# rsinghlab/GNN-Tumor-Seg

Hardware: AMD Instinct MI355X
Metric: supervoxel-graphs/sec training, 7xSAGE-pool-256, 15k-node graphs (higher is better)
Workload: dtype f32; 1 GPU; C2: 7xGraphSAGE-pool-256 (8 SAGEConv), fwd+weighted-CE+bwd+AdamW, 4 x 15000-node/86350-edge lattice graphs per GPU, 4-chan feat, fp32; global_batch=4, nodes_per_batch=60000, edges_per_batch=345400, parallelism=dp1

## Files before the change

gnn-tumor-seg_amd/csrc/gts_options.hip:

```cpp
#include "gts_gemm_args.h"
#include "gts_rows.h"

namespace gts {
namespace {

struct Option { int32_t id; int* knob; bool (*legal)(int32_t); };

const Option kOptions[] = {
    {GTS_OPT_GEMM_TILE, &g_fwd_variant, [](int32_t v) { return v == -1 || v == -2 || v == 1 || v == 3 || v == 5 || v == 8 || v == 10; }},
    {GTS_OPT_IGRAD_TILE, &g_igrad_variant, [](int32_t v) { return v == -1 || v == 1 || v == 3 || v == 5 || v == 8 || v == 10; }},
    {GTS_OPT_WGRAD_TILE, &g_wgrad_variant, [](int32_t v) { return v == -1 || v == 1 || v == 2 || v == 4 || v == 6; }},
    {GTS_OPT_GEMM_SCHED, &g_gemm_sched, nullptr},
    {GTS_OPT_PANEL_ROWS, &g_panel_rows, nullptr},
    {GTS_OPT_SPMM_ROWS_PER_WAVE, &g_spmm_seq, nullptr},
    {GTS_OPT_SPMM_STREAMING, &g_spmm_nt, nullptr},
    {GTS_OPT_PROJECT_STREAMING, &g_project_nt, nullptr},
    {GTS_OPT_CLUSTER_STREAMING, &g_cluster_nt, nullptr},
    {GTS_OPT_CLUSTER_DEALING, &g_cluster_dealing, [](int32_t v) { return v >= 0 && v <= 2; }},
    {GTS_OPT_CLUSTER_RING, &g_cluster_ring, nullptr},
    {GTS_OPT_CLUSTER_PER_CU, &g_cluster_per_cu, nullptr},
    {GTS_OPT_CLUSTER_CONSUMERS, &g_cluster_consumers, nullptr},
    {GTS_OPT_GAT_WALK, &g_gat_walk, nullptr},
    {GTS_OPT_GAT_CLUSTER_WAVES, &g_gat_cluster_waves, nullptr},
    {GTS_OPT_GAT_CLUSTER_GROUP, &g_gat_cluster_group, nullptr},
    {GTS_OPT_GAT_CLUSTER_DEALING, &g_gat_cluster_dealing, [](int32_t v) { return v == 0 || v == 1; }},
};

const Option* find_option(int32_t id) {
  for (const Option& o : kOptions)
    if (o.id == id) return &o;
  return nullptr;
}

}
}

extern "C" int32_t gts_set_option(int32_t option, int32_t value) {
  const gts::Option* o = gts::find_option(option);
  if (o == nullptr || (o->legal != nullptr && !o->legal(value))) return GTS_ERR_ARGKIND;
  *o->knob = value;
  return GTS_OK;
}

extern "C" int32_t gts_get_option(int32_t option) {
  const gts::Option* o = gts::find_option(option);
  return o != nullptr ? *o->knob : INT32_MIN;
}
```

gnn-tumor-seg_amd/csrc/gts_rows.h:

```cpp
#pragma once
#include <type_traits>

#include "gts_common.h"

namespace gts {

constexpr int kUnroll = 8;

__device__ __forceinline__ float mad(float w, float v, float acc) { return __builtin_fmaf(w, v, acc); }

typedef float v2f __attribute__((ext_vector_type(2)));
constexpr float kEluSplit = -0.35f, kLog2e = 1.44269504088896340736f;
constexpr float kEluC2 = 0.5f, kEluC3 = 1.0f / 6.0f, kEluC4 = 1.0f / 24.0f, kEluC5 = 1.0f / 120.0f, kEluC6 = 1.0f / 720.0f,
                kEluC7 = 1.0f / 5040.0f;
__device__ __forceinline__ float elu_expm1(float x) {
  float q = __builtin_fmaf(kEluC7, x, kEluC6);
  q = __builtin_fmaf(q, x, kEluC5);
  q = __builtin_fmaf(q, x, kEluC4);
  q = __builtin_fmaf(q, x, kEluC3);
  q = __builtin_fmaf(q, x, kEluC2);
  const float small = __builtin_fmaf(x * x, q, x);
  const float large = __builtin_amdgcn_exp2f(x * kLog2e) - 1.0f;
  return x < kEluSplit ? large : small;
}
// ... 29 lines not shown
    body(active ? c : 0, active);
  }
}

template <int N>
using IC = std::integral_constant<int, N>;

template <int LPR, typename Body>
__device__ __forceinline__ void for_chunks(int beg, int end, Body&& body) {
  if constexpr (LPR == kWave) {
    int k = beg;
    for (; k + kUnroll <= end; k += kUnroll) body(IC<kUnroll>{}, k);
    switch (end - k) {
      case 1: body(IC<1>{}, k); break;
      case 2: body(IC<2>{}, k); break;
      case 3: body(IC<3>{}, k); break;
      case 4: body(IC<4>{}, k); break;
      case 5: body(IC<5>{}, k); break;
      case 6: body(IC<6>{}, k); break;
      case 7: body(IC<7>{}, k); break;
      default: break;
    }
  } else {
    for (int k = beg; k < end; k += kUnroll) body(IC<kUnroll>{}, k);
  }
}

template <int LPR, int CNT>
struct Chunk {
  int reg;
  const int32_t* __restrict__ p;
  int k, last;
  __device__ __forceinline__ Chunk(const int32_t* __restrict__ arr, int k_, int end) : p(arr), k(k_), last(end - 1) {
    if constexpr (LPR == kWave) {
      const int lane = threadIdx.x & (kWave - 1);
      reg = lane < CNT ? arr[k_ + lane] : 0;
    } else {
      reg = 0;
    }
  }
  __device__ __forceinline__ int operator[](int j) const {
    if constexpr (LPR == kWave) {
      return __builtin_amdgcn_readlane(reg, j);
    } else {
      return p[min(k + j, last)];
    }
  }
  __device__ __forceinline__ bool valid(int j) const {
    if constexpr (LPR == kWave) return true;
    return k + j <= last;
  }
};

inline int g_spmm_seq = 0;
inline int g_project_nt = 1;
inline int g_spmm_nt = -1;
inline int g_cluster_nt = -1;
inline int g_gat_walk = 1;
inline int g_cluster_ring = 0;
inline int g_cluster_per_cu = 0;
inline int g_gat_cluster_waves = 0;
inline int g_cluster_dealing = 0;
inline int g_gat_cluster_dealing = 0;
inline int g_gat_cluster_group = 0;
inline int g_cluster_consumers = 0;

inline int pick_seq(int64_t n_rows, int rows_per_wave_step, int preferred) {
  if (g_spmm_seq > 0) return g_spmm_seq;
  if (preferred > 0) return preferred;
  const int64_t steps = (n_rows + rows_per_wave_step - 1) / rows_per_wave_step;
  int seq = 1;
  while (seq < 4 && steps / (seq * 2) >= 8192) seq *= 2;
  return seq;
}

struct Geometry {
  int vec, lpr, seq;
  dim3 grid;
};

inline Geometry make_geometry(int64_t n_rows, int64_t n_feat, int preferred_seq = 0) {
  Geometry g;
  g.vec = (n_feat % 4 == 0) ? 4 : 1;
  g.lpr = lanes_per_row(n_feat / g.vec);
  const int rows_per_step = kWave / g.lpr;
  g.seq = pick_seq(n_rows, rows_per_step, preferred_seq);
  const int64_t rows_per_block = static_cast<int64_t>(rows_per_step) * g.seq * kWavesPerBlock;
  g.grid = dim3(static_cast<unsigned>((n_rows + rows_per_block - 1) / rows_per_block));
  return g;
}

inline bool bad_shape(int64_t n_rows, int64_t n_feat) {
  return n_rows < 0 || n_feat <= 0 || n_rows >= (1LL << 31) || n_feat >= (1LL << 24);
}

}

#define GTS_DISPATCH_LPR(VEC_, LPR_VAL, ...)                \
  switch (LPR_VAL) {                                        \
    case 1: { constexpr int LPR = 1; __VA_ARGS__; } break;  \
    case 2: { constexpr int LPR = 2; __VA_ARGS__; } break;  \
    case 4: { constexpr int LPR = 4; __VA_ARGS__; } break;  \
    case 8: { constexpr int LPR = 8; __VA_ARGS__; } break;  \
    case 16: { constexpr int LPR = 16; __VA_ARGS__; } break; \
    case 32: { constexpr int LPR = 32; __VA_ARGS__; } break; \
    default: { constexpr int LPR = 64; __VA_ARGS__; } break; \
  }

#define GTS_DISPATCH_GEOM(G, ...)                                   \
  if ((G).vec == 4) {                                               \
    constexpr int VEC = 4;                                          \
    GTS_DISPATCH_LPR(4, (G).lpr, __VA_ARGS__)                       \
  } else {                                                          \
    constexpr int VEC = 1;                                          \
    GTS_DISPATCH_LPR(1, (G).lpr, __VA_ARGS__)                       \
  }
```

gnn-tumor-seg_amd/csrc/gts_spmm.hip:

```cpp
#include "gts_rows.h"

namespace gts {
namespace {

template <int ARGB>
struct ArgTraits;
template <>
struct ArgTraits<1> {
  using T = uint8_t;
  static constexpr int kNone = 0xFF;
};
template <>
struct ArgTraits<4> {
  using T = int32_t;
  static constexpr int kNone = -1;
};

template <int VEC, int ARGB>
__device__ __forceinline__ void store_slots(void* arg, size_t off, const int (&slot)[VEC]) {
  if constexpr (ARGB == 1) {
    uint8_t* p = static_cast<uint8_t*>(arg) + off;
    if constexpr (VEC == 4) {
      const uint32_t w = (slot[0] & 0xFF) | ((slot[1] & 0xFF) << 8) | ((slot[2] & 0xFF) << 16) |
                         (static_cast<uint32_t>(slot[3] & 0xFF) << 24);
      *reinterpret_cast<uint32_t*>(p) = w;
    } else {
      p[0] = static_cast<uint8_t>(slot[0]);
    }
  } else if constexpr (ARGB == 4) {
    int32_t* p = static_cast<int32_t*>(arg) + off;
    if constexpr (VEC == 4) {
      *reinterpret_cast<int4*>(p) = make_int4(slot[0], slot[1], slot[2], slot[3]);
    } else {
      p[0] = slot[0];
    }
  }
}

template <int VEC, int ARGB>
__device__ __forceinline__ void load_slots(const void* arg, size_t off, int (&slot)[VEC]) {
  if constexpr (ARGB == 1) {
    const uint8_t* p = static_cast<const uint8_t*>(arg) + off;
    if constexpr (VEC == 4) {
      const uint32_t w = *reinterpret_cast<const uint32_t*>(p);
      slot[0] = w & 0xFF;
      slot[1] = (w >> 8) & 0xFF;
      slot[2] = (w >> 16) & 0xFF;
      slot[3] = w >> 24;
    } else {
      slot[0] = p[0];
    }
  } else {
    const int32_t* p = static_cast<const int32_t*>(arg) + off;
    if constexpr (VEC == 4) {
      const int4 w = *reinterpret_cast<const int4*>(p);
      slot[0] = w.x, slot[1] = w.y, slot[2] = w.z, slot[3] = w.w;
    } else {
      slot[0] = p[0];
    }
  }
}

template <int VEC, int LPR, int ARGB>
__global__ __launch_bounds__(kBlock) void spmm_max_fwd_kernel(
    const int32_t* __restrict__ indptr, const int32_t* __restrict__ indices,
    const float* __restrict__ x, float* __restrict__ out, void* __restrict__ arg, int n_dst,
    int n_feat, int seq, int nt, int relu_input) {
  for (int s = 0; s < seq; ++s) {
    const int v = owned_row<LPR>(s, seq, n_dst);
    if (v < 0) continue;
    const int beg = indptr[v], end = indptr[v + 1];
    for_columns<VEC, LPR>(n_feat, [&](int c, bool active) {
      float best[VEC];
      int slot[VEC];
#pragma unroll
      for (int t = 0; t < VEC; ++t) best[t] = -INFINITY, slot[t] = -1;
      for_chunks<LPR>(beg, end, [&](auto cnt_c, int k) {
        constexpr int CNT = decltype(cnt_c)::value;
        const Chunk<LPR, CNT> src(indices, k, end);
        Vec<VEC> val[CNT];
#pragma unroll
        for (int j = 0; j < CNT; ++j)
          val[j] = Vec<VEC>::load(x + static_cast<size_t>(src[j]) * n_feat + c);
#pragma unroll
        for (int j = 0; j < CNT; ++j) {
          if (src.valid(j)) {
#pragma unroll
            for (int t = 0; t < VEC; ++t) {
              if (best[t] < val[j].v[t]) best[t] = val[j].v[t], slot[t] = k + j - beg;
            }
          }
        }
      });
      Vec<VEC> o;
#pragma unroll
      for (int t = 0; t < VEC; ++t) {
        const bool dead = isinf(best[t]);
        o.v[t] = dead ? 0.0f : best[t];
        slot[t] = (dead || (relu_input && !(best[t] > 0.0f))) ? -1 : slot[t];
      }
      const size_t off = static_cast<size_t>(v) * n_feat + c;
      if (active) {
        if (nt & 1) o.store_nt(out + off); else o.store(out + off);
        if constexpr (ARGB != 0) store_slots<VEC, ARGB>(arg, off, slot);
      }
    });
  }
}

template <int VEC, int LPR, int ARGB>
__global__ __launch_bounds__(kBlock) void spmm_max_bwd_kernel(
    const int32_t* __restrict__ t_indptr, const int32_t* __restrict__ t_indices,
    const int32_t* __restrict__ t_slot, const float* __restrict__ gout,
    const void* __restrict__ arg, const float* __restrict__ relu_src, float* __restrict__ gx,
    int n_src, int n_feat, int seq, int nt) {
  for (int s = 0; s < seq; ++s) {
    const int u = owned_row<LPR>(s, seq, n_src);
    if (u < 0) continue;
    const int beg = t_indptr[u], end = t_indptr[u + 1];
    for_columns<VEC, LPR>(n_feat, [&](int c, bool active) {
      float acc[VEC];
#pragma unroll
      for (int t = 0; t < VEC; ++t) acc[t] = 0.0f;
      for_chunks<LPR>(beg, end, [&](auto cnt_c, int k) {
        constexpr int CNT = decltype(cnt_c)::value;
        const Chunk<LPR, CNT> dst(t_indices, k, end);
        const Chunk<LPR, CNT> slt(t_slot, k, end);
        Vec<VEC> g[CNT];
        int win[CNT][VEC];
        int want[CNT];
#pragma unroll
        for (int j = 0; j < CNT; ++j) {
          const size_t off = static_cast<size_t>(dst[j]) * n_feat + c;
          want[j] = slt[j];
          g[j] = Vec<VEC>::load(gout + off);
          load_slots<VEC, ARGB>(arg, off, win[j]);
        }
#pragma unroll
        for (int j = 0; j < CNT; ++j) {
          if (dst.valid(j)) {
#pragma unroll
            for (int t = 0; t < VEC; ++t) acc[t] += (win[j][t] == want[j]) ? g[j].v[t] : 0.0f;
          }
        }
      });
      const size_t off = static_cast<size_t>(u) * n_feat + c;
      Vec<VEC> o;
      if (relu_src != nullptr) {
        const Vec<VEC> p = (nt & 2) ? Vec<VEC>::load_nt(relu_src + off) : Vec<VEC>::load(relu_src + off);
#pragma unroll
        for (int t = 0; t < VEC; ++t) o.v[t] = p.v[t] > 0.0f ? acc[t] : 0.0f;
      } else {
#pragma unroll
        for (int t = 0; t < VEC; ++t) o.v[t] = acc[t];
      }
      if (active) { if (nt & 1) o.store_nt(gx + off); else o.store(gx + off); }
    });
  }
}

constexpr int kLowRank = 4, kLowRankFeat = 256;

template <int ARGB>
__global__ __launch_bounds__(kBlock) void spmm_max_bwd_lowrank_kernel(
    const int32_t* __restrict__ t_indptr, const int32_t* __restrict__ t_indices,
    const int32_t* __restrict__ t_slot, const float* __restrict__ g, const float* __restrict__ w,
    const void* __restrict__ arg, float* __restrict__ gx, int n_src, int nt) {
  constexpr int VEC = 4, LPR = kWave, R = kLowRank, F = kLowRankFeat;
  const int u = owned_row<LPR>(0, 1, n_src);
  if (u < 0) return;
  const int c = VEC * (threadIdx.x & (kWave - 1));
  Vec<VEC> wk[R];
#pragma unroll
  for (int k = 0; k < R; ++k) wk[k] = Vec<VEC>::load(w + k * F + c);
  const int beg = t_indptr[u], end = t_indptr[u + 1];
  float acc[VEC];
#pragma unroll
  for (int t = 0; t < VEC; ++t) acc[t] = 0.0f;
  for_chunks<LPR>(beg, end, [&](auto cnt_c, int k) {
    constexpr int CNT = decltype(cnt_c)::value;
    const Chunk<LPR, CNT> dst(t_indices, k, end);
    const Chunk<LPR, CNT> slt(t_slot, k, end);
    Vec<R> gr[CNT];
    int win[CNT][VEC];
    int want[CNT];
#pragma unroll
    for (int j = 0; j < CNT; ++j) {
      const size_t d = static_cast<size_t>(dst[j]);
      want[j] = slt[j];
      gr[j] = Vec<R>::load(g + d * R);
      load_slots<VEC, ARGB>(arg, d * F + c, win[j]);
    }
#pragma unroll
    for (int j = 0; j < CNT; ++j) {
#pragma unroll
      for (int t = 0; t < VEC; ++t) {
        float v = 0.0f;
#pragma unroll
        for (int q = 0; q < R; ++q) v = __builtin_fmaf(gr[j].v[q], wk[q].v[t], v);
        acc[t] += (win[j][t] == want[j]) ? v : 0.0f;
      }
    }
  });
  Vec<VEC> o;
#pragma unroll
  for (int t = 0; t < VEC; ++t) o.v[t] = acc[t];
  const size_t off = static_cast<size_t>(u) * F + c;
  if (nt & 1) o.store_nt(gx + off); else o.store(gx + off);
}

template <int VEC, int LPR, bool DIV_IN>
__global__ __launch_bounds__(kBlock) void spmm_sum_kernel(
    const int32_t* __restrict__ indptr, const int32_t* __restrict__ indices,
    const float* __restrict__ x, float* __restrict__ out, const float* __restrict__ div_in,
    const float* __restrict__ div_out, const float* __restrict__ accum, int add_self, int n_out, int n_feat,
    int seq) {
  for (int s = 0; s < seq; ++s) {
    const int v = owned_row<LPR>(s, seq, n_out);
    if (v < 0) continue;
    const int beg = indptr[v], end = indptr[v + 1];
    for_columns<VEC, LPR>(n_feat, [&](int c, bool active) {
      float acc[VEC];
#pragma unroll
      for (int t = 0; t < VEC; ++t) acc[t] = 0.0f;
      for_chunks<LPR>(beg, end, [&](auto cnt_c, int k) {
        constexpr int CNT = decltype(cnt_c)::value;
        const Chunk<LPR, CNT> src(indices, k, end);
        Vec<VEC> val[CNT];
        float d[CNT];
#pragma unroll
        for (int j = 0; j < CNT; ++j) {
          const int u = src[j];
          d[j] = DIV_IN ? div_in[u] : 1.0f;
          val[j] = Vec<VEC>::load(x + static_cast<size_t>(u) * n_feat + c);
        }
#pragma unroll
        for (int j = 0; j < CNT; ++j) {
          if (src.valid(j)) {
#pragma unroll
            for (int t = 0; t < VEC; ++t) acc[t] += DIV_IN ? val[j].v[t] / d[j] : val[j].v[t];
          }
        }
      });
      const size_t off = static_cast<size_t>(v) * n_feat + c;
      if (add_self) {
        const Vec<VEC> self = Vec<VEC>::load(x + off);
        const float d = DIV_IN ? div_in[v] : 1.0f;
#pragma unroll
        for (int t = 0; t < VEC; ++t) acc[t] += DIV_IN ? self.v[t] / d : self.v[t];
      }
      Vec<VEC> o;
      const float dv = div_out != nullptr ? div_out[v] : 1.0f;
#pragma unroll
      for (int t = 0; t < VEC; ++t) o.v[t] = div_out != nullptr ? acc[t] / dv : acc[t];
      if (accum != nullptr) {
        const Vec<VEC> other = Vec<VEC>::load(accum + off);
#pragma unroll
        for (int t = 0; t < VEC; ++t) o.v[t] = other.v[t] + o.v[t];
      }
      if (active) o.store(out + off);
    });
  }
}

}
}

extern "C" int32_t gts_spmm_max_fwd_f32(const int32_t* indptr, const int32_t* indices,
                                        const float* x, float* out, void* arg,
                                        int32_t arg_bytes, int32_t relu_input, int64_t n_dst,
                                        int64_t n_feat, void* stream) {
  using namespace gts;
  if (!indptr || !x || !out || (arg_bytes != 0 && !arg)) return GTS_ERR_NULL;
  if (bad_shape(n_dst, n_feat)) return GTS_ERR_SHAPE;
  if (arg_bytes != 0 && arg_bytes != 1 && arg_bytes != 4) return GTS_ERR_ARGKIND;
  if (n_dst == 0) return GTS_OK;
  const Geometry g = make_geometry(n_dst, n_feat, 2);
  const int nt = g_spmm_nt < 0 ? 1 : g_spmm_nt;
  hipStream_t st = static_cast<hipStream_t>(stream);
  const int nd = static_cast<int>(n_dst), nf = static_cast<int>(n_feat);
  GTS_DISPATCH_GEOM(g, {
    if (arg_bytes == 0)
      spmm_max_fwd_kernel<VEC, LPR, 0><<<g.grid, kBlock, 0, st>>>(indptr, indices, x, out, arg, nd, nf, g.seq, nt, relu_input);
    else if (arg_bytes == 1)
      spmm_max_fwd_kernel<VEC, LPR, 1><<<g.grid, kBlock, 0, st>>>(indptr, indices, x, out, arg, nd, nf, g.seq, nt, relu_input);
    else
      spmm_max_fwd_kernel<VEC, LPR, 4><<<g.grid, kBlock, 0, st>>>(indptr, indices, x, out, arg, nd, nf, g.seq, nt, relu_input);
  })
  return launch_status();
}

extern "C" int32_t gts_spmm_max_bwd_f32(const int32_t* t_indptr, const int32_t* t_indices,
                                        const int32_t* t_slot, const float* gout,
                                        const void* arg, int32_t arg_bytes,
                                        const float* relu_src, float* gx, int64_t n_src,
                                        int64_t n_feat, void* stream) {
  using namespace gts;
  if (!t_indptr || !gout || !arg || !gx) return GTS_ERR_NULL;
  if (bad_shape(n_src, n_feat)) return GTS_ERR_SHAPE;
  if (arg_bytes != 1 && arg_bytes != 4) return GTS_ERR_ARGKIND;
  if (n_src == 0) return GTS_OK;
  const Geometry g = make_geometry(n_src, n_feat, 1);
  const int nt = g_spmm_nt < 0 ? 0 : g_spmm_nt;
  hipStream_t st = static_cast<hipStream_t>(stream);
  const int ns = static_cast<int>(n_src), nf = static_cast<int>(n_feat);
  GTS_DISPATCH_GEOM(g, {
    if (arg_bytes == 1)
      spmm_max_bwd_kernel<VEC, LPR, 1><<<g.grid, kBlock, 0, st>>>(t_indptr, t_indices, t_slot, gout, arg, relu_src, gx, ns, nf, g.seq, nt);
    else
      spmm_max_bwd_kernel<VEC, LPR, 4><<<g.grid, kBlock, 0, st>>>(t_indptr, t_indices, t_slot, gout, arg, relu_src, gx, ns, nf, g.seq, nt);
  })
  return launch_status();
}

extern "C" int32_t gts_spmm_max_bwd_lowrank_f32(const int32_t* t_indptr, const int32_t* t_indices,
                                                const int32_t* t_slot, const float* g, const float* w,
                                                const void* arg, int32_t arg_bytes, float* gx, int64_t n_src,
                                                int64_t n_feat, int64_t rank, void* stream) {
  using namespace gts;
  if (!t_indptr || !g || !w || !arg || !gx) return GTS_ERR_NULL;
  if (bad_shape(n_src, n_feat) || n_feat != kLowRankFeat || rank != kLowRank) return GTS_ERR_SHAPE;
  if (arg_bytes != 1 && arg_bytes != 4) return GTS_ERR_ARGKIND;
  if (n_src == 0) return GTS_OK;
  const int nt = g_spmm_nt < 0 ? 0 : g_spmm_nt;
  hipStream_t st = static_cast<hipStream_t>(stream);
  const unsigned grid = static_cast<unsigned>((n_src + kWavesPerBlock - 1) / kWavesPerBlock);
  const int ns = static_cast<int>(n_src);
  if (arg_bytes == 1)
    spmm_max_bwd_lowrank_kernel<1><<<grid, kBlock, 0, st>>>(t_indptr, t_indices, t_slot, g, w, arg, gx, ns, nt);
  else
    spmm_max_bwd_lowrank_kernel<4><<<grid, kBlock, 0, st>>>(t_indptr, t_indices, t_slot, g, w, arg, gx, ns, nt);
  return launch_status();
}

extern "C" int32_t gts_spmm_sum_f32(const int32_t* indptr, const int32_t* indices,
                                    const float* x, float* out, const float* div_in,
                                    const float* div_out, const float* accum, int32_t add_self,
                                    int64_t n_out, int64_t n_feat, void* stream) {
  using namespace gts;
  if (!indptr || !x || !out) return GTS_ERR_NULL;
  if (bad_shape(n_out, n_feat)) return GTS_ERR_SHAPE;
  if (n_out == 0) return GTS_OK;
  const Geometry g = make_geometry(n_out, n_feat);
  hipStream_t st = static_cast<hipStream_t>(stream);
  const int no = static_cast<int>(n_out), nf = static_cast<int>(n_feat);
  GTS_DISPATCH_GEOM(g, {
    if (div_in != nullptr)
      spmm_sum_kernel<VEC, LPR, true><<<g.grid, kBlock, 0, st>>>(indptr, indices, x, out, div_in, div_out, accum, add_self, no, nf, g.seq);
    else
      spmm_sum_kernel<VEC, LPR, false><<<g.grid, kBlock, 0, st>>>(indptr, indices, x, out, div_in, div_out, accum, add_self, no, nf, g.seq);
  })
  return launch_status();
}
```

gnn-tumor-seg_amd/gts/ops.py:

```python
import ctypes

import torch

from . import _lib
from ._lib import check, current_stream, ptr, require_device
from ._operands import StreamBuffers, expect, f32, scratch
from .graph import _DeviceSchedule

_ARG_DTYPE = {0: torch.uint8, 1: torch.uint8, 4: torch.int32}

KERNEL_TIMERS = {}
INSTRUMENTED = False


def _timed(name, launch):
    timer = KERNEL_TIMERS.get(name)
    return timer(launch) if timer is not None else launch()


_counters = StreamBuffers(torch.int32, zeroed=True)
_COUNTER_BYTES = 4 * _lib.const("GTS_CLUSTER_COUNTER_WORDS")


def cluster_counters(device):
# ... 38 lines not shown
    return g.dev_schedule(which)


def spmm_max_bwd(g, gout, arg, relu_src=None):
    gout = gout.contiguous()
    f32(gout, relu_src)
    require_device(gout, arg, relu_src)
    d = g.dev()
    if gout.dim() != 2 or gout.shape[0] != g.n:
        raise _lib.GtsError(f"gradient must be [graph nodes = {g.n}, F], got {tuple(gout.shape)}")
    n, f = g.n, gout.shape[1]
    expect(arg, (n, f), "arg")
    expect(relu_src, (n, f), "relu_src")
    if arg.dtype != _ARG_DTYPE[g.arg_bytes]:
        raise _lib.GtsError(f"arg dtype {arg.dtype} does not belong to this graph ({_ARG_DTYPE[g.arg_bytes]})")
    gx = torch.empty((n, f), dtype=torch.float32, device=gout.device)
    lib = _lib.load()
    ds = _cluster_schedule(g, "out", n, f, arg.element_size()) if relu_src is None else None
    if ds is not None:
        def launch():
            return lib.gts_spmm_max_bwd_cluster_f32(*_DeviceSchedule.launch_args(ds), ptr(gout), ptr(arg), 1, ptr(gx), n, f,
                                                    ptr(cluster_counters(gout.device)), current_stream())
    else:
        def launch():
            return lib.gts_spmm_max_bwd_f32(ptr(d.t_indptr), ptr(d.t_indices), ptr(d.t_slot), ptr(gout),
                                            ptr(arg), arg.element_size(), ptr(relu_src), ptr(gx), n, f,
                                            current_stream())

    check(_timed("spmm_max_bwd_f256", launch) if f == 256 else launch(), "gts_spmm_max_bwd_f32")
    return gx


def lowrank_bwd_applies(grad, w, arg):
    return grad.shape[1] == 4 and tuple(w.shape) == (4, 256) and arg.element_size() == 1


def spmm_max_bwd_lowrank(g, grad, w, arg):
    grad, w = grad.contiguous(), w.contiguous()
    f32(grad, w)
    require_device(grad, w, arg)
    d = g.dev()
    n = g.n
    if grad.dim() != 2 or grad.shape != (n, 4) or tuple(w.shape) != (4, 256):
        raise _lib.GtsError(f"spmm_max_bwd_lowrank takes a gradient [graph nodes = {n}, 4] and weights [4, 256], "
                            f"got {tuple(grad.shape)} and {tuple(w.shape)}")
    expect(arg, (n, 256), "arg")
    if arg.dtype != _ARG_DTYPE[g.arg_bytes]:
        raise _lib.GtsError(f"arg dtype {arg.dtype} does not belong to this graph ({_ARG_DTYPE[g.arg_bytes]})")
    gx = torch.empty((n, 256), dtype=torch.float32, device=grad.device)
    check(_lib.load().gts_spmm_max_bwd_lowrank_f32(ptr(d.t_indptr), ptr(d.t_indices), ptr(d.t_slot), ptr(grad), ptr(w),
                                                   ptr(arg), arg.element_size(), ptr(gx), n, 256, 4, current_stream()),
          "gts_spmm_max_bwd_lowrank_f32")
    return gx


def spmm_sum_raw(g, x, transposed=False, div_in=None, div_out=None, add_self=False, accum=None):
    x = x.contiguous()
    f32(x, div_in, div_out, accum)
    require_device(x, div_in, div_out, accum)
    d = g.dev()
    indptr, indices = (d.t_indptr, d.t_indices) if transposed else (d.indptr, d.indices)
    n = g.n
    if x.dim() != 2 or x.shape[0] != n:
        raise _lib.GtsError(f"features must be [graph nodes = {n}, F], got {tuple(x.shape)}")
    f = x.shape[1]
    expect(div_in, (n,), "div_in")
    expect(div_out, (n,), "div_out")
    expect(accum, (n, f), "accum")
    out = torch.empty_like(x)
    check(_lib.load().gts_spmm_sum_f32(ptr(indptr), ptr(indices), ptr(x), ptr(out), ptr(div_in), ptr(div_out),
                                       ptr(accum), 1 if add_self else 0, n, f, current_stream()), "gts_spmm_sum_f32")
    return out


class _SpMMMax(torch.autograd.Function):
    @staticmethod
    def forward(ctx, g, x):
        out, arg = spmm_max_fwd(g, x, want_arg=True)
        ctx.g = g
        ctx.save_for_backward(arg)
        return out

    @staticmethod
    def backward(ctx, gout):
        (arg,) = ctx.saved_tensors
        return None, spmm_max_bwd(ctx.g, gout, arg)


class _SpMMReduce(torch.autograd.Function):

    @staticmethod
    def forward(ctx, g, x, mode):
        ctx.g, ctx.mode = g, mode
        d = g.dev()
        if mode == "sum":
            return spmm_sum_raw(g, x)
        if mode == "mean":
            return spmm_sum_raw(g, x, div_out=d.deg_clamped)
        if mode == "gcn":
            return spmm_sum_raw(g, x, div_out=d.deg_plus1, add_self=True)
        raise ValueError(mode)

    @staticmethod
    def backward(ctx, gout):
        g, mode = ctx.g, ctx.mode
        d = g.dev()
# ... 1012 lines not shown
```

include/gts_hip.h:

```cpp
#ifndef GTS_HIP_H
#define GTS_HIP_H

#include <stdint.h>

#ifdef __cplusplus
extern "C" {
#endif

#define GTS_OK 0
#define GTS_ERR_NULL (-1)
#define GTS_ERR_SHAPE (-2)
#define GTS_ERR_ARGKIND (-3)

int32_t gts_abi_version(void);
const char* gts_error_string(int32_t code);

int32_t gts_spmm_max_fwd_f32(const int32_t* indptr, const int32_t* indices, const float* x,
                             float* out, void* arg, int32_t arg_bytes, int32_t relu_input,
                             int64_t n_dst, int64_t n_feat, void* stream);

int32_t gts_spmm_max_bwd_f32(const int32_t* t_indptr, const int32_t* t_indices,
                             const int32_t* t_slot, const float* gout, const void* arg,
                             int32_t arg_bytes, const float* relu_src, float* gx,
                             int64_t n_src, int64_t n_feat, void* stream);
int32_t gts_spmm_max_bwd_lowrank_f32(const int32_t* t_indptr, const int32_t* t_indices,
                                     const int32_t* t_slot, const float* g, const float* w, const void* arg,
                                     int32_t arg_bytes, float* gx, int64_t n_src, int64_t n_feat,
                                     int64_t rank, void* stream);

int64_t gts_cluster_record_words(int32_t max_rows, int32_t max_srcs, int32_t loc_words, int32_t with_tag);
int32_t gts_cluster_schedule(const int32_t* indptr, const int32_t* indices, const int32_t* t_indptr,
                             const int32_t* t_indices, const int32_t* edge_tag, int64_t n_rows,
                             int32_t max_rows, int32_t max_srcs, int32_t max_edges, int32_t* rec,
                             int64_t rec_capacity, int64_t* n_clusters, int64_t* n_staged,
                             int32_t* max_cluster_edges);
int64_t gts_cluster_lds_bytes(int32_t max_rows, int32_t max_srcs, int32_t loc_words, int32_t kind);
int32_t gts_spmm_max_fwd_cluster_f32(const int32_t* rec, int64_t n_clusters, int32_t max_rows, int32_t max_srcs,
                                     int32_t loc_words, const float* x, float* out, void* arg,
                                     int32_t arg_bytes, int32_t relu_input, int64_t n_rows, int64_t n_feat,
                                     uint32_t* counters, void* stream);
int32_t gts_spmm_max_bwd_cluster_f32(const int32_t* rec, int64_t n_clusters, int32_t max_rows, int32_t max_srcs,
                                     int32_t loc_words, const float* gout, const void* arg, int32_t arg_bytes,
                                     float* gx, int64_t n_rows, int64_t n_feat, uint32_t* counters, void* stream);
#define GTS_CLUSTER_COUNTER_WORDS 256
int32_t gts_cluster_uses_counters(int64_t n_clusters, int32_t max_rows, int32_t max_srcs, int32_t loc_words, int32_t backward);

int32_t gts_spmm_sum_f32(const int32_t* indptr, const int32_t* indices, const float* x,
                         float* out, const float* div_in, const float* div_out, const float* accum,
                         int32_t add_self, int64_t n_out, int64_t n_feat, void* stream);

int32_t gts_gat_fwd_f32(const int32_t* indptr, const int32_t* indices, const float* ft,
                        const float* el, const float* er, float negative_slope, const float* bias,
                        const float* residual, int32_t activation, float* out, float* attn,
                        int64_t n, int64_t heads, int64_t dim, void* stream);
int32_t gts_gat_scores_f32(const float* ft, const float* attn_l, const float* attn_r, float* el,
                           float* er, int64_t n, int64_t heads, int64_t dim, void* stream);

int32_t gts_gat_bwd_edge_f32(const int32_t* indptr, const int32_t* indices, const float* ft,
                             const float* el, const float* er, const float* attn,
                             const float* gout, float negative_slope, float* ge, float* ger,
                             int64_t n, int64_t heads, int64_t dim, void* stream);
int32_t gts_gat_bwd_src_f32(const int32_t* t_indptr, const int32_t* t_indices,
                            const int32_t* t_pos, const float* attn, const float* ge,
                            const float* gout, const float* attn_l, const float* attn_r,
                            const float* ger, float* gft, float* gel, int64_t n, int64_t heads,
                            int64_t dim, void* stream);
int64_t gts_gat_reduce_workspace(int64_t n, int64_t cols);
int32_t gts_gat_act_bwd_f32(const float* gout, const float* out, int32_t activation, float* g_pre,
                            float* g_bias, float* workspace, int64_t workspace_bytes, int64_t n,
                            int64_t cols, void* stream);
int32_t gts_gat_param_grad_f32(const float* ft, const float* gel, const float* ger, float* g_attn_l,
                               float* g_attn_r, float* workspace, int64_t workspace_bytes, int64_t n,
                               int64_t heads, int64_t dim, void* stream);

int64_t gts_gat_cluster_workspace(int64_t n_clusters, int32_t max_rows, int32_t loc_words, int64_t heads, int32_t backward);
int32_t gts_gat_attn_f32(const int32_t* indptr, const int32_t* indices, const float* el, const float* er,
                         float negative_slope, float* attn, int64_t n, int64_t heads, int64_t max_degree, void* stream);
int32_t gts_gat_fwd_cluster_f32(const int32_t* indptr, const int32_t* indices, const int32_t* rec, int64_t n_clusters,
                                int32_t max_rows, int32_t max_srcs, int32_t loc_words, int32_t tagged, const float* ft,
                                const float* el, const float* er, float negative_slope, const float* bias,
                                int32_t activation, float* out, float* attn, float* workspace, int64_t workspace_bytes,
// ... 130 lines not shown
                                        const float* const* params, int64_t n_rows, const int64_t* widths,
                                        int32_t n_layers, int32_t arg_bytes, int32_t relu_bits, const void* fwd_arena,
                                        float* const* grads, float* gx, void* scratch, int64_t scratch_bytes,
                                        int32_t top_done, void* stream);

int64_t gts_weighted_ce_workspace(int64_t n);
int32_t gts_weighted_ce_f32(const float* logits, const int64_t* labels, const float* class_w,
                            float* grad_unscaled, float* workspace, int64_t workspace_bytes,
                            float* out3, int64_t n, int64_t n_classes, void* stream);

#define GTS_DICE_CE_MAX_GROUPS 8
#define GTS_DICE_CE_STATS_FLOATS 40
#define GTS_DICE_CE_STATS_LOSS 0
#define GTS_DICE_CE_STATS_CE 1
#define GTS_DICE_CE_STATS_LDICE 2
#define GTS_DICE_CE_STATS_CE_NUM 3
#define GTS_DICE_CE_STATS_CE_DEN 4
#define GTS_DICE_CE_STATS_DICE 8
#define GTS_DICE_CE_STATS_I 16
#define GTS_DICE_CE_STATS_S 24
#define GTS_DICE_CE_STATS_T 32
int64_t gts_dice_ce_workspace(int64_t n, int32_t n_groups);
int32_t gts_dice_ce_fwd_f32(const float* logits, const int64_t* labels, const float* class_w,
                            const uint32_t* group_masks, int32_t n_groups, double ce_weight,
                            double dice_weight, double smooth, float* stats, void* workspace,
                            int64_t workspace_bytes, int64_t n, int64_t n_classes, void* stream);
int32_t gts_dice_ce_bwd_f32(const float* logits, const int64_t* labels, const float* class_w,
                            const uint32_t* group_masks, int32_t n_groups, double ce_weight,
                            double dice_weight, double smooth, const float* stats,
                            const float* grad_scale, float* grad, int64_t n, int64_t n_classes,
                            void* stream);

int32_t gts_augment_crop_f32(const float* x, const int64_t* labels, const float* params, float* x_out,
                             int64_t* labels_out, int64_t cx, int64_t cy, int64_t cz, int64_t channels,
                             int64_t image_channels, int32_t flip_mask, uint64_t seed, uint64_t step,
                             void* stream);
int32_t gts_augment_features_f32(const float* feats, const int64_t* row_ptr, const int64_t* row_ptr_host,
                                 const float* params, float* out, int64_t n_rows, int64_t n_feats,
                                 int64_t modalities, int64_t n_graphs, double sigma, uint64_t seed,
                                 uint64_t step, void* stream);

int32_t gts_augment_spatial_f32(const float* x, const int64_t* labels, const float* params,
                                const double* matrix, float* x_out, int64_t* labels_out, int64_t cx,
                                int64_t cy, int64_t cz, int64_t channels, int64_t image_channels,
                                int32_t flip_mask, uint64_t seed, uint64_t step, void* stream);
int32_t gts_augment_spatial_bwd_f32(const float* dy, const double* matrix, float* dx, int64_t cx, int64_t cy,
                                    int64_t cz, int64_t channels, int32_t flip_mask, void* stream);

#define GTS_OPT_GEMM_TILE 1
#define GTS_OPT_WGRAD_TILE 2
#define GTS_OPT_IGRAD_TILE 3
#define GTS_OPT_PROJECT_STREAMING 6
#define GTS_OPT_SPMM_ROWS_PER_WAVE 4
#define GTS_OPT_SPMM_STREAMING 5
#define GTS_OPT_GEMM_SCHED 7
#define GTS_OPT_CLUSTER_STREAMING 8
#define GTS_OPT_GAT_WALK 14
#define GTS_OPT_GAT_CLUSTER_WAVES 15
#define GTS_OPT_GAT_CLUSTER_GROUP 16
#define GTS_OPT_GAT_CLUSTER_DEALING 17
#define GTS_OPT_CLUSTER_DEALING 18
#define GTS_OPT_PANEL_ROWS 13
#define GTS_OPT_CLUSTER_RING 10
#define GTS_OPT_CLUSTER_PER_CU 11
#define GTS_OPT_CLUSTER_CONSUMERS 12
int32_t gts_set_option(int32_t option, int32_t value);
int32_t gts_get_option(int32_t option);

#define GTS_COLLATE_MAX_SCHEDULES 6
typedef struct {
  int64_t n_nodes, n_edges;
  const int32_t *indptr, *indices, *t_indptr, *t_indices, *t_slot, *t_pos;
  const void* features;
  const void* labels;
  int32_t feat_bytes;
  int32_t label_bytes;
  const int32_t* sched_rec[GTS_COLLATE_MAX_SCHEDULES];
  int64_t sched_clusters[GTS_COLLATE_MAX_SCHEDULES];
  int32_t sched_loc_words[GTS_COLLATE_MAX_SCHEDULES];
} gts_collate_member_t;
typedef struct {
  int32_t max_rows, max_srcs, tagged, reserved;
} gts_collate_kind_t;
typedef struct {
  int64_t total_bytes, n_nodes, n_edges;
  int64_t features, labels;
  int64_t csr[8];
  int64_t sched[GTS_COLLATE_MAX_SCHEDULES];
  int64_t sched_clusters[GTS_COLLATE_MAX_SCHEDULES];
  int32_t sched_loc_words[GTS_COLLATE_MAX_SCHEDULES];
  int32_t sched_record_words[GTS_COLLATE_MAX_SCHEDULES];
} gts_collate_plan_t;
int32_t gts_collate_plan(const gts_collate_member_t* members, int32_t n_members, int64_t feat_width,
                         const gts_collate_kind_t* kinds, int32_t n_kinds, gts_collate_plan_t* plan);
int32_t gts_collate_batch(const gts_collate_member_t* members, int32_t n_members, int64_t feat_width,
                          const gts_collate_kind_t* kinds, int32_t n_kinds, void* dst, int64_t dst_bytes,
                          int32_t n_threads, gts_collate_plan_t* plan);

#define GTS_GG_MAX_SV 32767
#define GTS_GG_MAX_K 32
#define GTS_GG_MAX_RADIUS 16
int32_t gts_gg_gaussian_f64(const double* in, double* out, double* tmp, const double* weights, int32_t radius,
                            double scale, int64_t d, int64_t h, int64_t w, int64_t c, void* stream);
int32_t gts_gg_slic_assign_f64(const double* img, const double* centres, int32_t n_centres, int64_t d, int64_t h,
                               int64_t w, int64_t c, int32_t step_z, int32_t step_y, int32_t step_x,
                               double spatial_weight, int32_t* labels, uint64_t* best, uint32_t* winner,
// ... 141 lines not shown
```

Baseline: 978.1 graphs/s.

## Add batched wave-row walk for 256-wide max-pool SpMM forward and backward

```diff
diff --git a/gnn-tumor-seg_amd/csrc/gts_options.hip b/gnn-tumor-seg_amd/csrc/gts_options.hip
--- a/gnn-tumor-seg_amd/csrc/gts_options.hip
+++ b/gnn-tumor-seg_amd/csrc/gts_options.hip
@@ -13,6 +13,7 @@
     {GTS_OPT_GEMM_SCHED, &g_gemm_sched, nullptr},
     {GTS_OPT_PANEL_ROWS, &g_panel_rows, nullptr},
     {GTS_OPT_SPMM_ROWS_PER_WAVE, &g_spmm_seq, nullptr},
+    {GTS_OPT_SPMM_WALK, &g_spmm_walk, [](int32_t v) { return v >= 0 && v <= 2; }},
     {GTS_OPT_SPMM_STREAMING, &g_spmm_nt, nullptr},
     {GTS_OPT_PROJECT_STREAMING, &g_project_nt, nullptr},
     {GTS_OPT_CLUSTER_STREAMING, &g_cluster_nt, nullptr},
diff --git a/gnn-tumor-seg_amd/csrc/gts_rows.h b/gnn-tumor-seg_amd/csrc/gts_rows.h
--- a/gnn-tumor-seg_amd/csrc/gts_rows.h
+++ b/gnn-tumor-seg_amd/csrc/gts_rows.h
@@ -105,6 +105,34 @@
   }
 };
 
+constexpr int kMaxBatchedSeq = kWave - 1;
+
+struct WaveRows {
+  int row0, count, ext;
+  __device__ __forceinline__ WaveRows(const int32_t* __restrict__ indptr, int seq, int n_rows) {
+    const int lane = threadIdx.x & (kWave - 1);
+    const int wave = threadIdx.x / kWave;
+    const int tile = xcd_contiguous_tile(blockIdx.x, gridDim.x);
+    row0 = __builtin_amdgcn_readfirstlane((tile * kWavesPerBlock + wave) * seq);
+    count = min(seq, n_rows - row0);
+    ext = count > 0 ? indptr[row0 + min(lane, count)] : 0;
+  }
+  __device__ __forceinline__ int extent(int s) const { return __builtin_amdgcn_readlane(ext, s); }
+};
+
+__device__ __forceinline__ int run_ids(const int32_t* __restrict__ arr, int beg0, int total) {
+  const int lane = threadIdx.x & (kWave - 1);
+  return lane < total ? arr[beg0 + lane] : 0;
+}
+
+__device__ __forceinline__ void settle_run(int reg) { asm volatile("" ::"s"(__builtin_amdgcn_readlane(reg, 0))); }
+
+struct RunChunk {
+  int reg, at;
+  __device__ __forceinline__ int operator[](int j) const { return __builtin_amdgcn_readlane(reg, at + j); }
+  __device__ __forceinline__ bool valid(int) const { return true; }
+};
+
 inline int g_spmm_seq = 0;
 inline int g_project_nt = 1;
 inline int g_spmm_nt = -1;
@@ -127,6 +155,23 @@
   return seq;
 }
 
+inline int g_spmm_walk = 0;
+
+struct Walk { int walk, seq; };
+constexpr int kSeqPerRow[3] = {2, 1, 1}, kSeqBatched[3] = {2, 2, 4};
+constexpr bool kBatchedByDefault[3] = {true, false, true};
+
+inline Walk pick_walk(int64_t n_rows, int64_t n_feat, int arg_bytes, int kind) {
+  const bool eligible = n_feat == 256 && n_rows > 0 && g_spmm_seq <= kMaxBatchedSeq &&
+                        (kind == 0 ? (arg_bytes == 0 || arg_bytes == 1 || arg_bytes == 4) : (arg_bytes == 1 || arg_bytes == 4));
+  const bool batched = eligible && (g_spmm_walk == 2 || (g_spmm_walk == 0 && kBatchedByDefault[kind]));
+  if (batched) return Walk{2, g_spmm_seq > 0 ? g_spmm_seq : kSeqBatched[kind]};
+  if (kind == 2) return Walk{1, 1};
+  const int vec = (n_feat % 4 == 0) ? 4 : 1;
+  const int rows_per_step = n_feat > 0 ? kWave / lanes_per_row(n_feat / vec) : 1;
+  return Walk{1, pick_seq(n_rows, rows_per_step, kSeqPerRow[kind])};
+}
+
 struct Geometry {
   int vec, lpr, seq;
   dim3 grid;
diff --git a/gnn-tumor-seg_amd/csrc/gts_spmm.hip b/gnn-tumor-seg_amd/csrc/gts_spmm.hip
--- a/gnn-tumor-seg_amd/csrc/gts_spmm.hip
+++ b/gnn-tumor-seg_amd/csrc/gts_spmm.hip
@@ -61,6 +61,47 @@
   }
 }
 
+template <int VEC, int LPR, int ARGB, typename MakeChunk>
+__device__ __forceinline__ void max_fwd_row(int v, int beg, int end, int n_feat, const float* __restrict__ x,
+                                            float* __restrict__ out, void* __restrict__ arg, int nt, int relu_input,
+                                            MakeChunk&& chunk) {
+  for_columns<VEC, LPR>(n_feat, [&](int c, bool active) {
+    float best[VEC];
+    int slot[VEC];
+#pragma unroll
+    for (int t = 0; t < VEC; ++t) best[t] = -INFINITY, slot[t] = -1;
+    for_chunks<LPR>(beg, end, [&](auto cnt_c, int k) {
+      constexpr int CNT = decltype(cnt_c)::value;
+      const auto src = chunk(cnt_c, k);
+      Vec<VEC> val[CNT];
+#pragma unroll
+      for (int j = 0; j < CNT; ++j)
+        val[j] = Vec<VEC>::load(x + static_cast<size_t>(src[j]) * n_feat + c);
+#pragma unroll
+      for (int j = 0; j < CNT; ++j) {
+        if (src.valid(j)) {
+#pragma unroll
+          for (int t = 0; t < VEC; ++t) {
+            if (best[t] < val[j].v[t]) best[t] = val[j].v[t], slot[t] = k + j - beg;
+          }
+        }
+      }
+    });
+    Vec<VEC> o;
+#pragma unroll
+    for (int t = 0; t < VEC; ++t) {
+      const bool dead = isinf(best[t]);
+      o.v[t] = dead ? 0.0f : best[t];
+      slot[t] = (dead || (relu_input && !(best[t] > 0.0f))) ? -1 : slot[t];
+    }
+    const size_t off = static_cast<size_t>(v) * n_feat + c;
+    if (active) {
+      if (nt & 1) o.store_nt(out + off); else o.store(out + off);
+      if constexpr (ARGB != 0) store_slots<VEC, ARGB>(arg, off, slot);
+    }
+  });
+}
+
 template <int VEC, int LPR, int ARGB>
 __global__ __launch_bounds__(kBlock) void spmm_max_fwd_kernel(
     const int32_t* __restrict__ indptr, const int32_t* __restrict__ indices,
@@ -70,42 +111,82 @@
     const int v = owned_row<LPR>(s, seq, n_dst);
     if (v < 0) continue;
     const int beg = indptr[v], end = indptr[v + 1];
-    for_columns<VEC, LPR>(n_feat, [&](int c, bool active) {
-      float best[VEC];
-      int slot[VEC];
-#pragma unroll
-      for (int t = 0; t < VEC; ++t) best[t] = -INFINITY, slot[t] = -1;
-      for_chunks<LPR>(beg, end, [&](auto cnt_c, int k) {
-        constexpr int CNT = decltype(cnt_c)::value;
-        const Chunk<LPR, CNT> src(indices, k, end);
-        Vec<VEC> val[CNT];
-#pragma unroll
-        for (int j = 0; j < CNT; ++j)
-          val[j] = Vec<VEC>::load(x + static_cast<size_t>(src[j]) * n_feat + c);
-#pragma unroll
-        for (int j = 0; j < CNT; ++j) {
-          if (src.valid(j)) {
-#pragma unroll
-            for (int t = 0; t < VEC; ++t) {
-              if (best[t] < val[j].v[t]) best[t] = val[j].v[t], slot[t] = k + j - beg;
-            }
-          }
+    max_fwd_row<VEC, LPR, ARGB>(v, beg, end, n_feat, x, out, arg, nt, relu_input, [&](auto cnt_c, int k) {
+      return Chunk<LPR, decltype(cnt_c)::value>(indices, k, end);
+    });
+  }
+}
+
+constexpr int kBatchedFeat = 256;
+constexpr int kBatchedWavesPerSimd = 8;
+
+template <int ARGB>
+__global__ __launch_bounds__(kBlock, kBatchedWavesPerSimd) void spmm_max_fwd_batched_kernel(
+    const int32_t* __restrict__ indptr, const int32_t* __restrict__ indices,
+    const float* __restrict__ x, float* __restrict__ out, void* __restrict__ arg, int n_dst, int seq, int nt,
+    int relu_input) {
+  constexpr int VEC = 4, LPR = kWave, F = kBatchedFeat;
+  const WaveRows rows(indptr, seq, n_dst);
+  if (rows.count <= 0) return;
+  const int beg0 = rows.extent(0), total = rows.extent(rows.count) - beg0;
+  if (total <= kWave) {
+    const int ids = run_ids(indices, beg0, total);
+    settle_run(ids);
+    for (int s = 0; s < rows.count; ++s)
+      max_fwd_row<VEC, LPR, ARGB>(rows.row0 + s, rows.extent(s), rows.extent(s + 1), F, x, out, arg, nt, relu_input,
+                                  [&](auto, int k) { return RunChunk{ids, k - beg0}; });
+  } else {
+    for (int s = 0; s < rows.count; ++s) {
+      const int end = rows.extent(s + 1);
+      max_fwd_row<VEC, LPR, ARGB>(rows.row0 + s, rows.extent(s), end, F, x, out, arg, nt, relu_input, [&](auto cnt_c, int k) {
+        return Chunk<LPR, decltype(cnt_c)::value>(indices, k, end);
+      });
+    }
+  }
+}
+
+template <int VEC, int LPR, int ARGB, typename MakeChunk>
+__device__ __forceinline__ void max_bwd_row(int u, int beg, int end, int n_feat, const float* __restrict__ gout,
+                                            const void* __restrict__ arg, const float* __restrict__ relu_src,
+                                            float* __restrict__ gx, int nt, MakeChunk&& chunk) {
+  for_columns<VEC, LPR>(n_feat, [&](int c, bool active) {
+    float acc[VEC];
+#pragma unroll
+    for (int t = 0; t < VEC; ++t) acc[t] = 0.0f;
+    for_chunks<LPR>(beg, end, [&](auto cnt_c, int k) {
+      constexpr int CNT = decltype(cnt_c)::value;
+      const auto dst = chunk(cnt_c, k, IC<0>{});
+      const auto slt = chunk(cnt_c, k, IC<1>{});
+      Vec<VEC> g[CNT];
+      int win[CNT][VEC];
+      int want[CNT];
+#pragma unroll
+      for (int j = 0; j < CNT; ++j) {
+        const size_t off = static_cast<size_t>(dst[j]) * n_feat + c;
+        want[j] = slt[j];
+        g[j] = Vec<VEC>::load(gout + off);
+        load_slots<VEC, ARGB>(arg, off, win[j]);
+      }
+#pragma unroll
+      for (int j = 0; j < CNT; ++j) {
+        if (dst.valid(j)) {
+#pragma unroll
+          for (int t = 0; t < VEC; ++t) acc[t] += (win[j][t] == want[j]) ? g[j].v[t] : 0.0f;
         }
-      });
-      Vec<VEC> o;
-#pragma unroll
-      for (int t = 0; t < VEC; ++t) {
-        const bool dead = isinf(best[t]);
-        o.v[t] = dead ? 0.0f : best[t];
-        slot[t] = (dead || (relu_input && !(best[t] > 0.0f))) ? -1 : slot[t];
-      }
-      const size_t off = static_cast<size_t>(v) * n_feat + c;
-      if (active) {
-        if (nt & 1) o.store_nt(out + off); else o.store(out + off);
-        if constexpr (ARGB != 0) store_slots<VEC, ARGB>(arg, off, slot);
       }
     });
-  }
+    const size_t off = static_cast<size_t>(u) * n_feat + c;
+    Vec<VEC> o;
+    if (relu_src != nullptr) {
+      const Vec<VEC> p = (nt & 2) ? Vec<VEC>::load_nt(relu_src + off) : Vec<VEC>::load(relu_src + off);
+#pragma unroll
+      for (int t = 0; t < VEC; ++t) o.v[t] = p.v[t] > 0.0f ? acc[t] : 0.0f;
+    } else {
+#pragma unroll
+      for (int t = 0; t < VEC; ++t) o.v[t] = acc[t];
+    }
+    if (active) { if (nt & 1) o.store_nt(gx + off); else o.store(gx + off); }
+  });
 }
 
 template <int VEC, int LPR, int ARGB>
@@ -118,48 +199,82 @@
     const int u = owned_row<LPR>(s, seq, n_src);
     if (u < 0) continue;
     const int beg = t_indptr[u], end = t_indptr[u + 1];
-    for_columns<VEC, LPR>(n_feat, [&](int c, bool active) {
-      float acc[VEC];
-#pragma unroll
-      for (int t = 0; t < VEC; ++t) acc[t] = 0.0f;
-      for_chunks<LPR>(beg, end, [&](auto cnt_c, int k) {
-        constexpr int CNT = decltype(cnt_c)::value;
-        const Chunk<LPR, CNT> dst(t_indices, k, end);
-        const Chunk<LPR, CNT> slt(t_slot, k, end);
-        Vec<VEC> g[CNT];
-        int win[CNT][VEC];
-        int want[CNT];
-#pragma unroll
-        for (int j = 0; j < CNT; ++j) {
-          const size_t off = static_cast<size_t>(dst[j]) * n_feat + c;
-          want[j] = slt[j];
-          g[j] = Vec<VEC>::load(gout + off);
-          load_slots<VEC, ARGB>(arg, off, win[j]);
-        }
-#pragma unroll
-        for (int j = 0; j < CNT; ++j) {
-          if (dst.valid(j)) {
-#pragma unroll
-            for (int t = 0; t < VEC; ++t) acc[t] += (win[j][t] == want[j]) ? g[j].v[t] : 0.0f;
-          }
-        }
-      });
-      const size_t off = static_cast<size_t>(u) * n_feat + c;
-      Vec<VEC> o;
-      if (relu_src != nullptr) {
-        const Vec<VEC> p = (nt & 2) ? Vec<VEC>::load_nt(relu_src + off) : Vec<VEC>::load(relu_src + off);
-#pragma unroll
-        for (int t = 0; t < VEC; ++t) o.v[t] = p.v[t] > 0.0f ? acc[t] : 0.0f;
-      } else {
-#pragma unroll
-        for (int t = 0; t < VEC; ++t) o.v[t] = acc[t];
+    max_bwd_row<VEC, LPR, ARGB>(u, beg, end, n_feat, gout, arg, relu_src, gx, nt, [&](auto cnt_c, int k, auto which) {
+      return Chunk<LPR, decltype(cnt_c)::value>(decltype(which)::value == 0 ? t_indices : t_slot, k, end);
+    });
+  }
+}
+
+template <int ARGB>
+__global__ __launch_bounds__(kBlock, ARGB == 1 ? kBatchedWavesPerSimd : 1) void spmm_max_bwd_batched_kernel(
+    const int32_t* __restrict__ t_indptr, const int32_t* __restrict__ t_indices,
+    const int32_t* __restrict__ t_slot, const float* __restrict__ gout,
+    const void* __restrict__ arg, const float* __restrict__ relu_src, float* __restrict__ gx,
+    int n_src, int seq, int nt) {
+  constexpr int VEC = 4, LPR = kWave, F = kBatchedFeat;
+  const WaveRows rows(t_indptr, seq, n_src);
+  if (rows.count <= 0) return;
+  const int beg0 = rows.extent(0), total = rows.extent(rows.count) - beg0;
+  if (total <= kWave) {
+    const int ids = run_ids(t_indices, beg0, total), slots = run_ids(t_slot, beg0, total);
+    settle_run(ids), settle_run(slots);
+    for (int s = 0; s < rows.count; ++s)
+      max_bwd_row<VEC, LPR, ARGB>(rows.row0 + s, rows.extent(s), rows.extent(s + 1), F, gout, arg, relu_src, gx, nt,
+                                  [&](auto, int k, auto which) {
+                                    return RunChunk{decltype(which)::value == 0 ? ids : slots, k - beg0};
+                                  });
+  } else {
+    for (int s = 0; s < rows.count; ++s) {
+      const int end = rows.extent(s + 1);
+      max_bwd_row<VEC, LPR, ARGB>(rows.row0 + s, rows.extent(s), end, F, gout, arg, relu_src, gx, nt,
+                                  [&](auto cnt_c, int k, auto which) {
+                                    return Chunk<LPR, decltype(cnt_c)::value>(decltype(which)::value == 0 ? t_indices : t_slot, k, end);
+                                  });
+    }
+  }
+}
+
+constexpr int kLowRank = 4, kLowRankFeat = 256;
+
+template <int ARGB, typename MakeChunk>
+__device__ __forceinline__ void lowrank_row(int u, int beg, int end, const Vec<4> (&wk)[kLowRank], const float* __restrict__ g,
+                                            const void* __restrict__ arg, float* __restrict__ gx, int nt, MakeChunk&& chunk) {
+  constexpr int VEC = 4, LPR = kWave, R = kLowRank, F = kLowRankFeat;
+  const int c = VEC * (threadIdx.x & (kWave - 1));
+  float acc[VEC];
+#pragma unroll
+  for (int t = 0; t < VEC; ++t) acc[t] = 0.0f;
+  for_chunks<LPR>(beg, end, [&](auto cnt_c, int k) {
+    constexpr int CNT = decltype(cnt_c)::value;
+    const auto dst = chunk(cnt_c, k, IC<0>{});
+    const auto slt = chunk(cnt_c, k, IC<1>{});
+    Vec<R> gr[CNT];
+    int win[CNT][VEC];
+    int want[CNT];
+#pragma unroll
+    for (int j = 0; j < CNT; ++j) {
+      const size_t d = static_cast<size_t>(dst[j]);
+      want[j] = slt[j];
+      gr[j] = Vec<R>::load(g + d * R);
+      load_slots<VEC, ARGB>(arg, d * F + c, win[j]);
+    }
+#pragma unroll
+    for (int j = 0; j < CNT; ++j) {
+#pragma unroll
+      for (int t = 0; t < VEC; ++t) {
+        float v = 0.0f;
+#pragma unroll
+        for (int q = 0; q < R; ++q) v = __builtin_fmaf(gr[j].v[q], wk[q].v[t], v);
+        acc[t] += (win[j][t] == want[j]) ? v : 0.0f;
       }
-      if (active) { if (nt & 1) o.store_nt(gx + off); else o.store(gx + off); }
-    });
-  }
-}
-
-constexpr int kLowRank = 4, kLowRankFeat = 256;
+    }
+  });
+  Vec<VEC> o;
+#pragma unroll
+  for (int t = 0; t < VEC; ++t) o.v[t] = acc[t];
+  const size_t off = static_cast<size_t>(u) * F + c;
+  if (nt & 1) o.store_nt(gx + off); else o.store(gx + off);
+}
 
 template <int ARGB>
 __global__ __launch_bounds__(kBlock) void spmm_max_bwd_lowrank_kernel(
@@ -174,39 +289,39 @@
 #pragma unroll
   for (int k = 0; k < R; ++k) wk[k] = Vec<VEC>::load(w + k * F + c);
   const int beg = t_indptr[u], end = t_indptr[u + 1];
-  float acc[VEC];
-#pragma unroll
-  for (int t = 0; t < VEC; ++t) acc[t] = 0.0f;
-  for_chunks<LPR>(beg, end, [&](auto cnt_c, int k) {
-    constexpr int CNT = decltype(cnt_c)::value;
-    const Chunk<LPR, CNT> dst(t_indices, k, end);
-    const Chunk<LPR, CNT> slt(t_slot, k, end);
-    Vec<R> gr[CNT];
-    int win[CNT][VEC];
-    int want[CNT];
-#pragma unroll
-    for (int j = 0; j < CNT; ++j) {
-      const size_t d = static_cast<size_t>(dst[j]);
-      want[j] = slt[j];
-      gr[j] = Vec<R>::load(g + d * R);
-      load_slots<VEC, ARGB>(arg, d * F + c, win[j]);
-    }
-#pragma unroll
-    for (int j = 0; j < CNT; ++j) {
-#pragma unroll
-      for (int t = 0; t < VEC; ++t) {
-        float v = 0.0f;
-#pragma unroll
-        for (int q = 0; q < R; ++q) v = __builtin_fmaf(gr[j].v[q], wk[q].v[t], v);
-        acc[t] += (win[j][t] == want[j]) ? v : 0.0f;
-      }
-    }
+  lowrank_row<ARGB>(u, beg, end, wk, g, arg, gx, nt, [&](auto cnt_c, int k, auto which) {
+    return Chunk<LPR, decltype(cnt_c)::value>(decltype(which)::value == 0 ? t_indices : t_slot, k, end);
   });
-  Vec<VEC> o;
-#pragma unroll
-  for (int t = 0; t < VEC; ++t) o.v[t] = acc[t];
-  const size_t off = static_cast<size_t>(u) * F + c;
-  if (nt & 1) o.store_nt(gx + off); else o.store(gx + off);
+}
+
+template <int ARGB>
+__global__ __launch_bounds__(kBlock) void spmm_max_bwd_lowrank_batched_kernel(
+    const int32_t* __restrict__ t_indptr, const int32_t* __restrict__ t_indices,
+    const int32_t* __restrict__ t_slot, const float* __restrict__ g, const float* __restrict__ w,
+    const void* __restrict__ arg, float* __restrict__ gx, int n_src, int seq, int nt) {
+  constexpr int VEC = 4, LPR = kWave, R = kLowRank, F = kLowRankFeat;
+  const WaveRows rows(t_indptr, seq, n_src);
+  if (rows.count <= 0) return;
+  const int c = VEC * (threadIdx.x & (kWave - 1));
+  Vec<VEC> wk[R];
+#pragma unroll
+  for (int k = 0; k < R; ++k) wk[k] = Vec<VEC>::load(w + k * F + c);
+  const int beg0 = rows.extent(0), total = rows.extent(rows.count) - beg0;
+  if (total <= kWave) {
+    const int ids = run_ids(t_indices, beg0, total), slots = run_ids(t_slot, beg0, total);
+    settle_run(ids), settle_run(slots);
+    for (int s = 0; s < rows.count; ++s)
+      lowrank_row<ARGB>(rows.row0 + s, rows.extent(s), rows.extent(s + 1), wk, g, arg, gx, nt, [&](auto, int k, auto which) {
+        return RunChunk{decltype(which)::value == 0 ? ids : slots, k - beg0};
+      });
+  } else {
+    for (int s = 0; s < rows.count; ++s) {
+      const int end = rows.extent(s + 1);
+      lowrank_row<ARGB>(rows.row0 + s, rows.extent(s), end, wk, g, arg, gx, nt, [&](auto cnt_c, int k, auto which) {
+        return Chunk<LPR, decltype(cnt_c)::value>(decltype(which)::value == 0 ? t_indices : t_slot, k, end);
+      });
+    }
+  }
 }
 
 template <int VEC, int LPR, bool DIV_IN>
@@ -263,7 +378,22 @@
   }
 }
 
-}
+inline unsigned batched_grid(int64_t n_rows, int seq) {
+  const int64_t rows_per_block = static_cast<int64_t>(seq) * kWavesPerBlock;
+  return static_cast<unsigned>((n_rows + rows_per_block - 1) / rows_per_block);
+}
+
+}
+}
+
+extern "C" int32_t gts_spmm_walk_for(int64_t n_rows, int64_t n_feat, int32_t arg_bytes, int32_t backward) {
+  using namespace gts;
+  if (bad_shape(n_rows, n_feat)) return GTS_ERR_SHAPE;
+  if (backward < 0 || backward > 2) return GTS_ERR_ARGKIND;
+  if (arg_bytes != 1 && arg_bytes != 4 && !(arg_bytes == 0 && backward == 0)) return GTS_ERR_ARGKIND;
+  if (backward == 2 && n_feat != kLowRankFeat) return GTS_ERR_SHAPE;
+  const Walk walk = pick_walk(n_rows, n_feat, arg_bytes, backward);
+  return walk.walk * GTS_SPMM_WALK_STRIDE + walk.seq;
 }
 
 extern "C" int32_t gts_spmm_max_fwd_f32(const int32_t* indptr, const int32_t* indices,
@@ -275,10 +405,21 @@
   if (bad_shape(n_dst, n_feat)) return GTS_ERR_SHAPE;
   if (arg_bytes != 0 && arg_bytes != 1 && arg_bytes != 4) return GTS_ERR_ARGKIND;
   if (n_dst == 0) return GTS_OK;
-  const Geometry g = make_geometry(n_dst, n_feat, 2);
   const int nt = g_spmm_nt < 0 ? 1 : g_spmm_nt;
   hipStream_t st = static_cast<hipStream_t>(stream);
   const int nd = static_cast<int>(n_dst), nf = static_cast<int>(n_feat);
+  const Walk walk = pick_walk(n_dst, n_feat, arg_bytes, 0);
+  if (walk.walk == 2) {
+    const unsigned grid = batched_grid(n_dst, walk.seq);
+    if (arg_bytes == 0)
+      spmm_max_fwd_batched_kernel<0><<<grid, kBlock, 0, st>>>(indptr, indices, x, out, arg, nd, walk.seq, nt, relu_input);
+    else if (arg_bytes == 1)
+      spmm_max_fwd_batched_kernel<1><<<grid, kBlock, 0, st>>>(indptr, indices, x, out, arg, nd, walk.seq, nt, relu_input);
+    else
+      spmm_max_fwd_batched_kernel<4><<<grid, kBlock, 0, st>>>(indptr, indices, x, out, arg, nd, walk.seq, nt, relu_input);
+    return launch_status();
+  }
+  const Geometry g = make_geometry(n_dst, n_feat, kSeqPerRow[0]);
   GTS_DISPATCH_GEOM(g, {
     if (arg_bytes == 0)
       spmm_max_fwd_kernel<VEC, LPR, 0><<<g.grid, kBlock, 0, st>>>(indptr, indices, x, out, arg, nd, nf, g.seq, nt, relu_input);
@@ -300,10 +441,19 @@
   if (bad_shape(n_src, n_feat)) return GTS_ERR_SHAPE;
   if (arg_bytes != 1 && arg_bytes != 4) return GTS_ERR_ARGKIND;
   if (n_src == 0) return GTS_OK;
-  const Geometry g = make_geometry(n_src, n_feat, 1);
   const int nt = g_spmm_nt < 0 ? 0 : g_spmm_nt;
   hipStream_t st = static_cast<hipStream_t>(stream);
   const int ns = static_cast<int>(n_src), nf = static_cast<int>(n_feat);
+  const Walk walk = pick_walk(n_src, n_feat, arg_bytes, 1);
+  if (walk.walk == 2) {
+    const unsigned grid = batched_grid(n_src, walk.seq);
+    if (arg_bytes == 1)
+      spmm_max_bwd_batched_kernel<1><<<grid, kBlock, 0, st>>>(t_indptr, t_indices, t_slot, gout, arg, relu_src, gx, ns, walk.seq, nt);
+    else
+      spmm_max_bwd_batched_kernel<4><<<grid, kBlock, 0, st>>>(t_indptr, t_indices, t_slot, gout, arg, relu_src, gx, ns, walk.seq, nt);
+    return launch_status();
+  }
+  const Geometry g = make_geometry(n_src, n_feat, kSeqPerRow[1]);
   GTS_DISPATCH_GEOM(g, {
     if (arg_bytes == 1)
       spmm_max_bwd_kernel<VEC, LPR, 1><<<g.grid, kBlock, 0, st>>>(t_indptr, t_indices, t_slot, gout, arg, relu_src, gx, ns, nf, g.seq, nt);
@@ -324,8 +474,17 @@
   if (n_src == 0) return GTS_OK;
   const int nt = g_spmm_nt < 0 ? 0 : g_spmm_nt;
   hipStream_t st = static_cast<hipStream_t>(stream);
+  const int ns = static_cast<int>(n_src);
+  const Walk walk = pick_walk(n_src, n_feat, arg_bytes, 2);
+  if (walk.walk == 2) {
+    const unsigned grid = batched_grid(n_src, walk.seq);
+    if (arg_bytes == 1)
+      spmm_max_bwd_lowrank_batched_kernel<1><<<grid, kBlock, 0, st>>>(t_indptr, t_indices, t_slot, g, w, arg, gx, ns, walk.seq, nt);
+    else
+      spmm_max_bwd_lowrank_batched_kernel<4><<<grid, kBlock, 0, st>>>(t_indptr, t_indices, t_slot, g, w, arg, gx, ns, walk.seq, nt);
+    return launch_status();
+  }
   const unsigned grid = static_cast<unsigned>((n_src + kWavesPerBlock - 1) / kWavesPerBlock);
-  const int ns = static_cast<int>(n_src);
   if (arg_bytes == 1)
     spmm_max_bwd_lowrank_kernel<1><<<grid, kBlock, 0, st>>>(t_indptr, t_indices, t_slot, g, w, arg, gx, ns, nt);
   else
diff --git a/gnn-tumor-seg_amd/gts/ops.py b/gnn-tumor-seg_amd/gts/ops.py
--- a/gnn-tumor-seg_amd/gts/ops.py
+++ b/gnn-tumor-seg_amd/gts/ops.py
@@ -114,6 +114,18 @@
                                                    ptr(arg), arg.element_size(), ptr(gx), n, 256, 4, current_stream()),
           "gts_spmm_max_bwd_lowrank_f32")
     return gx
+
+
+_OPT_SPMM_WALK = _lib.const("GTS_OPT_SPMM_WALK")
+_WALK_STRIDE = _lib.const("GTS_SPMM_WALK_STRIDE")
+WALK_PER_ROW, WALK_BATCHED = 1, 2
+
+
+def spmm_walk_for(n_rows, n_feat, arg_bytes, backward=0):
+    code = _lib.load().gts_spmm_walk_for(n_rows, n_feat, arg_bytes, backward)
+    if code < 0:
+        check(code, "gts_spmm_walk_for")
+    return divmod(code, _WALK_STRIDE)
 
 
 def spmm_sum_raw(g, x, transposed=False, div_in=None, div_out=None, add_self=False, accum=None):
diff --git a/include/gts_hip.h b/include/gts_hip.h
--- a/include/gts_hip.h
+++ b/include/gts_hip.h
@@ -27,6 +27,8 @@
                                      const int32_t* t_slot, const float* g, const float* w, const void* arg,
                                      int32_t arg_bytes, float* gx, int64_t n_src, int64_t n_feat,
                                      int64_t rank, void* stream);
+#define GTS_SPMM_WALK_STRIDE 65536
+int32_t gts_spmm_walk_for(int64_t n_rows, int64_t n_feat, int32_t arg_bytes, int32_t backward);
 
 int64_t gts_cluster_record_words(int32_t max_rows, int32_t max_srcs, int32_t loc_words, int32_t with_tag);
 int32_t gts_cluster_schedule(const int32_t* indptr, const int32_t* indices, const int32_t* t_indptr,
@@ -263,6 +265,7 @@
 #define GTS_OPT_IGRAD_TILE 3
 #define GTS_OPT_PROJECT_STREAMING 6
 #define GTS_OPT_SPMM_ROWS_PER_WAVE 4
+#define GTS_OPT_SPMM_WALK (21)
 #define GTS_OPT_SPMM_STREAMING 5
 #define GTS_OPT_GEMM_SCHED 7
 #define GTS_OPT_CLUSTER_STREAMING 8
```

Measured after the change: 980.0 graphs/s (median of 5 runs). No clear change (+0.2%).
